# aksiksi/needle

Hardware: AMD Instinct MI355X
Metric: episode-pairs/sec (analyze+search) (higher is better)
Workload: dtype f64-certified (f32 first pass)

## Files before the change

needle_amd/csrc/common.h:

```cpp
#pragma once

#include <cstddef>
#include <cstdint>
#include <functional>
#include <string>
#include <vector>

#include "../../include/needle_hip.h"

struct ihipStream_t;

namespace needle {

struct Status {
  NeedleError code = NeedleError_Ok;
  std::string message;
  bool ok() const { return code == NeedleError_Ok; }
  static Status Ok() { return Status{}; }
  static Status Make(NeedleError c, std::string m) { return Status{c, std::move(m)}; }
};

NeedleError report(const Status &s);
void set_last_error(const std::string &m);
const char *last_error();
// ... 67 lines not shown
  uint64_t data_offset = 0;
  uint64_t frames = 0;
};
Status wav_probe(const std::string &path, WavInfo *out);
Status wav_read_frames(const std::string &path, const WavInfo &info, uint64_t first, uint64_t count, int16_t *dst);

struct StreamSpan {
  uint64_t pcm_off;
  uint64_t num_values;
  uint64_t item_off;
};

Status gpu_fingerprint_device(const int16_t *d_pcm, const std::vector<StreamSpan> &streams, int channels,
                              uint32_t step, uint32_t *d_items, bool sync, double *d_chroma_dbg = nullptr,
                              double *d_feat_dbg = nullptr, size_t descriptor_slot = 0, int pipe = -1,
                              uint32_t *zero_word = nullptr, bool *zeroed = nullptr);
Status gpu_fingerprint_streamed_device(const std::vector<const int16_t *> &pcm, const std::vector<size_t> &num_values,
                                       int channels, uint32_t step, uint32_t *d_items,
                                       const std::vector<uint64_t> &item_off);
Status gpu_fingerprint_host(const std::vector<const int16_t *> &pcm, const std::vector<size_t> &num_values,
                            int channels, uint32_t step, std::vector<std::vector<uint32_t>> *items,
                            int rate = kSampleRate);
using PcmReader = std::function<Status(size_t stream, uint64_t first_value, uint64_t num_values, int16_t *dst)>;
using StreamIssued = std::function<Status(size_t stream_index)>;
Status gpu_upload_pcm_streamed(const std::vector<size_t> &num_values, const std::vector<uint64_t> &dev_off,
                               const PcmReader &read, unsigned readers, int16_t *d_pcm, ::ihipStream_t *stream = nullptr,
                               const StreamIssued &issued = nullptr);
Status gpu_upload_pcm(const std::vector<const int16_t *> &pcm, const std::vector<size_t> &num_values,
                      const std::vector<uint64_t> &dev_off, int16_t *d_pcm, ::ihipStream_t *stream = nullptr,
                      const StreamIssued &issued = nullptr);
Status gpu_fingerprint_streamed(const std::vector<size_t> &num_values, const PcmReader &read, unsigned readers,
                                int channels, uint32_t step, std::vector<std::vector<uint32_t>> *items,
                                int rate = kSampleRate);
Status gpu_hamming_runs_device(const uint32_t *d_hashes, const NeedleHipSeq *seqs, size_t num_seqs,
                               const NeedleHipProblem *problems, size_t num_problems, uint32_t threshold,
                               NeedleHipRun *d_runs, uint32_t capacity, uint32_t *d_count, bool sync,
                               bool count_is_zero = false);
Status gpu_hamming_runs_host(const uint32_t *hashes, size_t num_hashes, const NeedleHipSeq *seqs, size_t num_seqs,
                             const NeedleHipProblem *problems, size_t num_problems, uint32_t threshold,
                             std::vector<NeedleHipRun> *runs);

uint32_t *gpu_pinned_arena_acquire(size_t words);
void gpu_pinned_arena_release(uint32_t *arena);
void gpu_prefetch_hashes(const uint32_t *hashes, size_t num_hashes);

constexpr uint64_t kDeviceEpiloguePairs = 1u << 14;
constexpr uint32_t kDeviceEpilogueRuns = 1u << 14;

Status gpu_int_valu_ceiling(double *cells_per_second);
Status gpu_scan_issued_evaluations(uint64_t *lane_evaluations, bool reset, uint64_t *head_survivors = nullptr);
void gpu_scan_last_launch(int32_t *form, uint64_t *matrix_products);
Status gpu_fingerprint_cert_stats(uint64_t out[4], bool reset);
Status gpu_fingerprint_audit_device(const int16_t *d_pcm, const std::vector<StreamSpan> &spans, int channels, uint32_t step,
                                    const uint32_t *d_items, uint64_t out[4], double *max_ratio, double *max_sigma);

struct ResampleSpan {
  uint64_t in_off;
  uint64_t n_in;
  uint64_t out_off;
};
size_t resample_out_len(size_t n_in, int rate);
Status gpu_resample_device(const int16_t *d_in, const std::vector<ResampleSpan> &spans, int channels, int rate,
                           int16_t *d_out, bool sync);
Status gpu_resample_host(const std::vector<const int16_t *> &pcm, const std::vector<size_t> &num_values, int channels,
                         int rate, std::vector<std::vector<int16_t>> *out);

struct DownmixSpan {
  const int16_t *src;
  int16_t *dst;
  uint64_t frames;
// ... 7 lines not shown
```

needle_amd/csrc/library.cpp:

```cpp
#include <hip/hip_runtime_api.h>

#include <algorithm>
#include <chrono>
#include <cstdio>
#include <cstdlib>
#include <cstring>
#include <map>
#include <new>
#include <tuple>

#include "comm.h"
#include "epilogue.h"
#include "hipctx.h"
#include "needle_core.h"

struct FrameHashes;
struct NeedleAudioComparator;

namespace needle {
const Comparator &comparator_of(const NeedleAudioComparator *c);
FrameHashes *make_frame_hashes(FrameHashesData &&d);
void fill_c_result(const VideoResult &v, NeedleHipSearchResult *r);
}

// ... 43 lines not shown
    DeviceBuffer<uint8_t> d_heads;
    uint32_t slab_runs = 0, head_runs = 0;
    int world = 0;
    void *host = nullptr;
    size_t host_bytes = 0;
    hipEvent_t searched = nullptr, done = nullptr;
    bool pending = false;
    std::vector<NeedleHipRun> merged;
    void *host_results = nullptr;
    size_t host_results_bytes = 0;
    bool device_epilogue = false, sharded = false;
    bool shape_fixed = false;
    const NeedleHipRun *last_runs = nullptr;
    size_t last_total = 0;
    DeviceBuffer<uint8_t> d_dir_send, d_dir_recv;
    DeviceBuffer<uint32_t> d_dir_counts;
    void *host_counts = nullptr;
    size_t host_counts_bytes = 0;
    std::vector<uint32_t> cap;
    bool ran_device_epilogue = false, ran_sharded = false;
    uint32_t scan_form = 0;
    bool counted = false;
    bool directed = false;
    std::vector<NeedleHipRun> fetched;
    bool fetched_valid = false;
    static size_t count_words(int world) { return ((size_t)world + 1 + 3) & ~(size_t)3; }
    uint64_t comm_bytes[4] = {0, 0, 0, 0};
    size_t slab_bytes() const { return kSlabHeader + (size_t)slab_runs * sizeof(NeedleHipRun); }
    size_t head_bytes() const { return kSlabHeader + (size_t)head_runs * sizeof(NeedleHipRun); }
  } job[2];
  static constexpr size_t kSlabHeader = 32;
  uint32_t slab_runs = 0;
  uint32_t last_max_count = 0;
  std::vector<uint32_t> dir_counts;
  int dir_world = 0;
  bool dir_unsupported = false;
  bool dir_cap_forced = false;
  size_t arena_rows = 0;
  const uint32_t *count_zeroed = nullptr;
  std::vector<uint32_t> row_len, row_ts;
  std::vector<uint64_t> row_seek, ts_tables;
  void ensure_row_tables() {
    if (row_len.size() == rows()) return;
    row_len.assign(rows(), 0);
    row_ts.assign(rows(), 0);
    row_seek.assign(rows(), 0);
    ts_tables.clear();
    std::map<uint32_t, uint32_t> offset_of;
    for (size_t row = 0; row < rows(); row++) {
      const Window &w = win[row];
      auto it = offset_of.find(w.kept);
      if (it == offset_of.end()) {
        it = offset_of.emplace(w.kept, (uint32_t)ts_tables.size()).first;
        for (const HashTs &h : timestamps(w.kept)) ts_tables.push_back(h.ts);
      }
      row_len[row] = w.kept;
      row_ts[row] = it->second;
      row_seek[row] = w.seek;
    }
  }
  ~NeedleHipLibrary() {
    for (Fetch &f : fetch) {
      if (f.host) (void)hipHostFree(f.host);
      if (f.done) (void)hipEventDestroy(f.done);
      if (f.ready) (void)hipEventDestroy(f.ready);
    }
// ... 359 lines not shown
      lib->problems_for[0] = ~(size_t)0;
    }
    std::vector<NeedleHipProblem> &problems = lib->problems;
    const bool cached = lib->problems_for[0] == first_pair && lib->problems_for[1] == num_pairs && lib->problems_for[2] == Rc;
    if (!cached) {
      lib->problems_for[0] = ~(size_t)0;
      problems.clear();
      problems.reserve(num_pairs * Rc);
      size_t i = 0, j = 0;
      if (num_pairs) pair_at(lib->n, first_pair, &i, &j);
      for (size_t p = first_pair; p < first_pair + num_pairs; p++) {
        for (size_t r = 0; r < Rc; r++) {
          if (r == 1 && (lib->win[i * R + 1].kept == 0 || lib->win[j * R + 1].kept == 0))
            return report(Status::Make(NeedleError_Unknown, "no ending hash data present"));
          const uint32_t a = lib->min_len[i * R + r], b = lib->min_len[j * R + r];
          if (a == 0 || b == 0) continue;
          problems.push_back(NeedleHipProblem{(uint32_t)(i * R + r), (uint32_t)(j * R + r), std::max(a, b),
                                              (uint32_t)(p * Rc + r)});
        }
        if (++j == lib->n) j = ++i + 1;
      }
      lib->problems_for[0] = first_pair;
      lib->problems_for[1] = num_pairs;
      lib->problems_for[2] = Rc;
    }
    for (NeedleHipLibrary::Fetch &f : lib->fetch)
      if (f.pending && (f.d_runs == d_runs || f.d_count == d_count) &&
          hipStreamWaitEvent(library_stream(), f.done, 0) != hipSuccess)
        return report(Status::Make(NeedleError_Unknown, "stream wait failed"));
    const auto t_built = std::chrono::steady_clock::now();
    const bool count_is_zero = lib->count_zeroed == d_count;
    lib->count_zeroed = nullptr;
    Status s = gpu_hamming_runs_device(lib->arena, seqs.data(), seqs.size(), problems.data(), problems.size(),
                                       cmp.hash_match_threshold(), d_runs, capacity, d_count, sync, count_is_zero);
    if (getenv("NEEDLE_HIP_TRACE"))
      std::fprintf(stderr, "[needle_hip] search enqueue: %zu problems built in %.2f ms, launched in %.2f ms\n",
                   problems.size(), std::chrono::duration<double, std::milli>(t_built - t_enter).count(),
                   std::chrono::duration<double, std::milli>(std::chrono::steady_clock::now() - t_built).count());
    return s.ok() ? NeedleError_Ok : report(s);
  });
}

enum NeedleError needle_hip_library_fetch_runs_begin(NeedleHipLibrary *lib, int slot, const NeedleHipRun *d_runs,
                                                     const uint32_t *d_count, uint32_t max_runs) {
  if (!lib || !d_runs || !d_count) return NeedleError_NullArgument;
  if (slot < 0 || slot > 1 || max_runs == 0) return NeedleError_InvalidArgument;
  return guarded([&]() -> NeedleError {
    NeedleHipLibrary::Fetch &f = lib->fetch[slot];
    if (f.pending) return report(Status::Make(NeedleError_InvalidArgument, "fetch slot still pending"));
    const size_t bytes = 16 + (size_t)max_runs * sizeof(NeedleHipRun);
    if (f.max_runs < max_runs) {
      if (f.host) (void)hipHostFree(f.host);
      f.host = nullptr;
      if (hipHostMalloc(&f.host, bytes, hipHostMallocDefault) != hipSuccess)
        return report(Status::Make(NeedleError_Unknown, "pinned allocation failed"));
      f.max_runs = max_runs;
    }
    if (!f.done && hipEventCreateWithFlags(&f.done, hipEventDisableTiming) != hipSuccess)
      return report(Status::Make(NeedleError_Unknown, "event creation failed"));
    if (!f.ready && hipEventCreateWithFlags(&f.ready, hipEventDisableTiming) != hipSuccess)
      return report(Status::Make(NeedleError_Unknown, "event creation failed"));
    hipStream_t stream = library_stream(), down = download_stream();
    if (hipEventRecord(f.ready, stream) != hipSuccess || hipStreamWaitEvent(down, f.ready, 0) != hipSuccess ||
        hipMemcpyAsync(f.host, d_count, sizeof(uint32_t), hipMemcpyDeviceToHost, down) != hipSuccess ||
        hipMemcpyAsync(static_cast<char *>(f.host) + 16, d_runs, (size_t)max_runs * sizeof(NeedleHipRun),
                       hipMemcpyDeviceToHost, down) != hipSuccess ||
        hipEventRecord(f.done, down) != hipSuccess)
// ... 152 lines not shown
}

bool device_epilogue_wanted(const NeedleHipLibrary *lib, size_t comparator_regions) {
  if (const char *e = getenv("NEEDLE_HIP_DEVICE_EPILOGUE")) return atoi(e) != 0;
  return (uint64_t)pair_count(lib->n) * comparator_regions >= kDeviceEpiloguePairs || lib->last_max_count >= kDeviceEpilogueRuns;
}

Status fetch_directed(NeedleHipLibrary::Job &j, int world, int rank) {
  if (j.fetched_valid) return Status::Ok();
  const size_t W = (size_t)world, cw = NeedleHipLibrary::Job::count_words(world);
  const uint32_t *m = static_cast<const uint32_t *>(j.host_counts);
  size_t total = 0, off = 0;
  for (size_t r = 0; r < W; r++) total += std::min(m[r * cw + 1 + (size_t)rank], j.cap[r * W + (size_t)rank]);
  j.fetched.resize(total);
  size_t at = 0;
  for (size_t r = 0; r < W; r++) {
    const uint32_t cap = j.cap[r * W + (size_t)rank], have = std::min(m[r * cw + 1 + (size_t)rank], cap);
    if (have)
      NEEDLE_HIP_TRY(hipMemcpyAsync(j.fetched.data() + at, j.d_dir_recv.ptr + off + NeedleHipLibrary::kSlabHeader,
                                    (size_t)have * sizeof(NeedleHipRun), hipMemcpyDeviceToHost, download_stream()));
    at += have;
    off += NeedleHipLibrary::kSlabHeader + (size_t)cap * sizeof(NeedleHipRun);
  }
  NEEDLE_HIP_TRY(hipStreamSynchronize(download_stream()));
  j.fetched_valid = true;
  return Status::Ok();
}

NeedleError job_search_and_gather(NeedleHipLibrary *lib, const NeedleAudioComparator *comparator, NeedleHipLibrary::Job &j) {
  const int world = comm_world(), rank = comm_rank();
  size_t pfirst = 0, pcount = 0;
  shard_range(pair_count(lib->n), world, rank, &pfirst, &pcount);
  uint8_t *mine = j.d_slabs.ptr;
  NeedleError e = needle_hip_library_search(lib, comparator, pfirst, pcount,
                                            reinterpret_cast<NeedleHipRun *>(mine + NeedleHipLibrary::kSlabHeader), j.slab_runs,
                                            reinterpret_cast<uint32_t *>(mine), false);
  if (e != NeedleError_Ok) return e;
  {
    int32_t form = 0;
    uint64_t products = 0;
    gpu_scan_last_launch(&form, &products);
    j.scan_form = (uint32_t)form;
  }
  hipStream_t stream = library_stream(), down = download_stream();
  if (hipEventRecord(j.searched, stream) != hipSuccess || hipStreamWaitEvent(down, j.searched, 0) != hipSuccess)
    return report(Status::Make(NeedleError_Unknown, "stream ordering failed"));
  const Comparator &cmp = comparator_of(comparator);
  const size_t Rc = cmp.include_endings() ? 2 : 1;
  j.device_epilogue = device_epilogue_wanted(lib, Rc) && lib->n >= 2;
  j.shape_fixed = j.device_epilogue;
  if (j.device_epilogue) {
    uint64_t shard_from = 1u << 16;
    if (const char *e = getenv("NEEDLE_HIP_SHARD_EPILOGUE_PAIRS")) shard_from = (uint64_t)std::max(1, atoi(e));
    j.sharded = world > 1 && (getenv("NEEDLE_HIP_SHARD_EPILOGUE") ? atoi(getenv("NEEDLE_HIP_SHARD_EPILOGUE")) != 0
                                                                   : (uint64_t)pair_count(lib->n) * Rc >= shard_from);
  }
  j.counted = j.directed = false;
  j.cap.clear();
  j.fetched_valid = false;
  const char *dir_env = getenv("NEEDLE_HIP_DIRECTED_RUNS");
  const bool want_directed = world > 1 && world <= 64 && j.device_epilogue && j.sharded && !lib->dir_unsupported &&
                             !(dir_env && atoi(dir_env) == 0);
  std::vector<size_t> recv_off((size_t)world, 0), recv_bytes((size_t)world, 0);
  if (want_directed) {
    const size_t W = (size_t)world;
    const bool have = lib->dir_world == world && lib->dir_counts.size() == W * W;
    std::vector<uint32_t> cap(W * W, 0u);
    if (have)
      for (size_t k = 0; k < W * W; k++) cap[k] = round_up4((uint64_t)lib->dir_counts[k] + lib->dir_counts[k] / 8 + 64);
// ... 505 lines not shown
```

needle_amd/csrc/search.hip:

```cpp
#include "epilogue.h"
#include "hipctx.h"

#include <algorithm>
#include <atomic>
#include <cstdio>
#include <cstdlib>
#include <cstring>
#include <mutex>
#include <unordered_map>

namespace needle {

namespace {

constexpr int kDiagsPerBlock = 256;
constexpr int kBandR = 7, kBandU = 3;
constexpr int kBandB = 64 * kBandR;
constexpr int kSampleW = 8;
constexpr int kSampleHead = 3;
__host__ __device__ constexpr int head_row(int k, int W, int H = kSampleHead) {
  return H == 3 ? (k == 0 ? 0 : (k == 1 ? W / 2 : W - 1)) : (k * (W - 1)) / (H - 1);
}
__host__ __device__ constexpr bool is_head_row(int s, int W, int H = kSampleHead) {
  for (int k = 0; k < H; k++)
// ... 148 lines not shown
      const uint32_t sv = src[row];
#pragma unroll
      for (int r = 0; r < R; r++) {
        const uint32_t c = (uint32_t)__popc(sv ^ W[(r + s) % R]);
        Z[r] = (c <= threshold) ? Z[r] : row;
        if (r == 0) W[s % R] = nxt[s];
      }
    }
    bool any = false;
#pragma unroll
    for (int r = 0; r < R; r++) any |= (i + K - 1 - Z[r] >= flag_len);
    if (__any(any)) checkpoint(i + K - 1);
  }
  for (; i <= i_end; i++) {
    const uint32_t sv = src[i];
#pragma unroll
    for (int r = 0; r < R; r++) {
      const uint32_t c = (uint32_t)__popc(sv ^ W[r]);
      Z[r] = (c <= threshold) ? Z[r] : i;
    }
#pragma unroll
    for (int r = 0; r + 1 < R; r++) W[r] = W[r + 1];
    W[R - 1] = lds[B + i + d_l + R];
  }
}

__device__ __forceinline__ void wave_lds_fence_search() {
  __builtin_amdgcn_fence(__ATOMIC_RELEASE, "wavefront");
  __builtin_amdgcn_wave_barrier();
  __builtin_amdgcn_fence(__ATOMIC_ACQUIRE, "wavefront");
}

template <int R, int W, bool COUNT = false, int H = kSampleHead, bool LEGACY = false>
__global__ __launch_bounds__(256) void hamming_runs_sampled_kernel(const uint32_t *__restrict__ hashes,
                                                                   const SearchProblem *__restrict__ problems,
                                                                   int num_problems, uint32_t threshold,
                                                                   NeedleHipRun *__restrict__ runs,
                                                                   uint32_t capacity, uint32_t *__restrict__ count,
                                                                   int bands_per_wave, int sparse_max,
                                                                   unsigned long long *__restrict__ eval_groups) {
  constexpr int B = 64 * R;
  unsigned long long groups = 0, survived = 0;
  extern __shared__ uint32_t lds[];
  __builtin_amdgcn_s_setprio(3);
  int lo = 0, hi = num_problems - 1;
  while (lo < hi) {
    int mid = (lo + hi + 1) >> 1;
    if (problems[mid].block_base <= blockIdx.x) lo = mid; else hi = mid - 1;
  }
  const SearchProblem pr = problems[lo];
  const int n = (int)pr.n, m = (int)pr.m;
  const uint32_t *__restrict__ src = hashes + pr.src_off;
  const uint32_t *__restrict__ dst = hashes + pr.dst_off;
  uint32_t *ldst = lds;
  for (int k = threadIdx.x; k < B; k += blockDim.x) {
    ldst[k] = 0u;
    ldst[B + m + k] = 0u;
  }
  {
    constexpr int kU = 8;
    const int nt = (int)blockDim.x;
    int k = threadIdx.x;
    for (; k + (kU - 1) * nt < m; k += kU * nt) {
      uint32_t v[kU];
#pragma unroll
      for (int u = 0; u < kU; u++) v[u] = dst[k + u * nt];
#pragma unroll
      for (int u = 0; u < kU; u++) ldst[B + k + u * nt] = v[u];
    }
    for (; k < m; k += nt) ldst[B + k] = dst[k];
  }
  const uint32_t *__restrict__ lsrc = src;
  __syncthreads();

  const int wave = __builtin_amdgcn_readfirstlane((int)(threadIdx.x >> 6));
  const int lane = (int)(threadIdx.x & 63);
  const int min_len = (int)pr.min_len;
  const int P = min_len - W + 1;
  const uint32_t bias = 31u - min(threshold, 31u);
  uint32_t held_b = 0u, held_e = 0u, held_len = 0u;
  int held = 0;
  auto flush_runs = [&]() {
    if (held == 0) return;
    uint32_t base = 0u;
    if (lane == 0) base = atomicAdd(count, (uint32_t)held);
    base = (uint32_t)__builtin_amdgcn_readfirstlane((int)base);
    if (lane < held && base + (uint32_t)lane < capacity)
      runs[base + (uint32_t)lane] = NeedleHipRun{(uint32_t)lo, held_b, held_e, held_len, 0u, 0u};
    held = 0;
  };
  auto emit_run = [&](const uint32_t b, const uint32_t e, const uint32_t len) {
    const bool mine = lane == held;
    held_b = mine ? b : held_b;
    held_e = mine ? e : held_e;
    held_len = mine ? len : held_len;
    if (++held == 64) flush_runs();
  };
  const int slots = 4 * bands_per_wave;
  const int total_bands = (n + m - 3 + B - 1) / B;
  const int nb = (total_bands + slots - 1) / slots;
  const int b_in_pair = (int)(blockIdx.x - pr.block_base);
  for (int round = 0; round < bands_per_wave; round++) {
  const int q = (round * 4 + wave + lo) % slots;
  const int band = q * nb + b_in_pair;
  const int D0 = band * B - (n - 2);
  if (band >= total_bands || D0 > m - 2) continue;
  const int i_start = max(1, 2 - D0 - B);
  const int i_end = min(n - 1, m - 1 - D0);
  const int d_l = D0 + lane * R;

  int k0 = (i_start - 1 + P - 1) / P;
  for (int w0 = 1 + k0 * P; w0 + W - 1 <= i_end; w0 += P) {
    uint32_t E[W + R - 1];
#pragma unroll
    for (int q = 0; q < W + R - 1; q++) E[q] = ldst[B + w0 + d_l + q];
    uint32_t sv[W];
#pragma unroll
    for (int s = 0; s < W; s++) sv[s] = src[w0 + s];
    bool ok[R];
    uint32_t miss[R];
#pragma unroll
    for (int r = 0; r < R; r++) miss[r] = 0u;
#pragma unroll
    for (int k = 0; k < H; k++) {
      const int s = head_row(k, W, H);
#pragma unroll
      for (int r = 0; r < R; r++) miss[r] |= (uint32_t)__popc(sv[s] ^ E[s + r]) + bias;
    }
#pragma unroll
    for (int r = 0; r < R; r++) ok[r] = miss[r] < 32u;
// ... 9 lines not shown
        const int row = e + lane;
        const bool bad = row <= fwd_limit && (uint32_t)__popc(lsrc[row] ^ ldst[B + row + d]) > threshold;
        if (COUNT) groups += 1;
        const unsigned long long mm = __ballot(bad);
        if (mm) {
          e += __ffsll((long long)mm) - 1;
          ended = true;
          break;
        }
        e += 64;
      }
      if (!ended) {
        if (fwd_limit == w0 + P + W - 1) return;
        e = ihi + 1;
      }
      const int b = e - 1;
      int a = ilo;
      int q = w0 - 1;
      while (q >= ilo) {
        const int row = q - lane;
        const bool bad = row >= ilo && (uint32_t)__popc(lsrc[row] ^ ldst[B + row + d]) > threshold;
        if (COUNT) groups += 1;
        const unsigned long long mm = __ballot(bad);
        if (mm) {
          a = q - (__ffsll((long long)mm) - 1) + 1;
          break;
        }
        q -= 64;
      }
      const int len = b - a + 1;
      if (len >= min_len) emit_run((uint32_t)b, (uint32_t)(b + d), (uint32_t)len);
    };

    unsigned long long alive[R];
    int survivors = 0;
#pragma unroll
    for (int r = 0; r < R; r++) {
      alive[r] = __ballot(ok[r]);
      survivors += __popcll(alive[r]);
    }
    if (COUNT) survived += (unsigned long long)survivors;
    if (survivors == 0) continue;
    if (!LEGACY || sparse_max < 0) {
#pragma unroll
      for (int r = 0; r < R; r++) {
        if (alive[r] == 0) continue;
        uint32_t mm = miss[r];
#pragma unroll
        for (int k = 0; k < W - H; k++) {
          const int s = tail_row(k, W, H);
          mm |= (uint32_t)__popc(sv[s] ^ E[s + r]) + bias;
        }
        if (COUNT) groups += W - H;
        unsigned long long cand = __ballot(mm < 32u);
        while (cand) {
          const int src_lane = __ffsll((long long)cand) - 1;
          cand &= cand - 1;
          resolve(D0 + src_lane * R + r);
        }
      }
      continue;
    }
    if constexpr (LEGACY) {
    if (survivors <= sparse_max) {
      constexpr int kTail = W - H;
      uint32_t sv_tail = sv[tail_row(kTail - 1, W, H)];
      int tail_off = tail_row(kTail - 1, W, H);
#pragma unroll
      for (int k = kTail - 2; k >= 0; k--) {
        sv_tail = lane == k ? sv[tail_row(k, W, H)] : sv_tail;
        tail_off = lane == k ? tail_row(k, W, H) : tail_off;
      }
#pragma unroll
      for (int r = 0; r < R; r++) {
        unsigned long long cand = alive[r];
        while (cand) {
          const int src_lane = __ffsll((long long)cand) - 1;
          cand &= cand - 1;
          const int d = D0 + src_lane * R + r;
          const int row = w0 + tail_off;
          const bool bad = (uint32_t)__popc(sv_tail ^ ldst[B + row + d]) > threshold;
          if (COUNT) groups += 1;
          if (__ballot(bad) == 0) resolve(d);
        }
      }
      continue;
    }
#pragma unroll
    for (int k = 0; k < W - H; k++) {
      const int s = tail_row(k, W, H);
// ... 104 lines not shown
    }
  }
}

struct ScanShape {
  int w = kSampleW, h = kSampleHead;
};
ScanShape scan_shape() {
  ScanShape sh;
  if (const char *e = getenv("NEEDLE_HIP_SCAN_SHAPE")) {
    int w = 0, h = 0;
    if (std::sscanf(e, "%d,%d", &w, &h) == 2 && (w == 4 || w == 8 || w == 16) && h >= 2 && h <= 4 && h < w) {
      sh.w = w;
      sh.h = h;
    }
  }
  return sh;
}
using SampledKernel = void (*)(const uint32_t *, const SearchProblem *, int, uint32_t, NeedleHipRun *, uint32_t, uint32_t *, int, int,
                               unsigned long long *);
template <bool COUNT>
SampledKernel sampled_kernel(ScanShape sh, bool legacy) {
#define NEEDLE_SHAPE(W_, H_) \
  if (sh.w == W_ && sh.h == H_) return hamming_runs_sampled_kernel<kBandR, W_, COUNT, H_, true>;
  NEEDLE_SHAPE(4, 2) NEEDLE_SHAPE(4, 3) NEEDLE_SHAPE(8, 2) NEEDLE_SHAPE(8, 4) NEEDLE_SHAPE(16, 2) NEEDLE_SHAPE(16, 3) NEEDLE_SHAPE(16, 4)
#undef NEEDLE_SHAPE
  if (legacy) return hamming_runs_sampled_kernel<kBandR, kSampleW, COUNT, kSampleHead, true>;
  return hamming_runs_sampled_kernel<kBandR, kSampleW, COUNT, kSampleHead, false>;
}

struct SearchPlan {
  std::vector<NeedleHipSeq> seqs;
  std::vector<NeedleHipProblem> problems;
  int mode[8] = {0, 0, 0, 0, 0, 0, 0, 0};
  std::vector<SearchProblem> meta;
  size_t staged = 0;
  uint64_t oversize_blocks = 0;
  uint64_t blocks = 0;
  size_t lds_bytes = 0;
  bool sampled = false, fast = false, mfma = false;
  int mfma_waves = 0, mfma_splits = 1;
  std::vector<M2ImageSeq> image_seqs;
  uint32_t image_windows = 0, image_min_len = 0;
  uint64_t mfma_products = 0;
  int bands_per_wave = 1;
  bool valid = false;
  bool matches(const NeedleHipSeq *s, size_t ns, const NeedleHipProblem *p, size_t np, const int *m) const {
    return valid && seqs.size() == ns && problems.size() == np && std::memcmp(mode, m, sizeof(mode)) == 0 &&
           std::memcmp(seqs.data(), s, ns * sizeof(NeedleHipSeq)) == 0 &&
           std::memcmp(problems.data(), p, np * sizeof(NeedleHipProblem)) == 0;
  }
};

int device_cus() {
  int cus = 256, dev = 0;
  if (hipGetDevice(&dev) == hipSuccess) (void)hipDeviceGetAttribute(&cus, hipDeviceAttributeMultiprocessorCount, dev);
  return cus > 0 ? cus : 256;
}

Status build_plan(const NeedleHipSeq *seqs, size_t num_seqs, const NeedleHipProblem *problems, size_t num_problems,
                  const int *mode, SearchPlan *plan) {
  plan->valid = false;
  std::vector<SearchProblem> &meta = plan->meta;
  meta.clear();
  meta.reserve(num_problems);
  uint64_t blocks = 0;
  for (size_t p = 0; p < num_problems; p++) {
    const NeedleHipProblem &pr = problems[p];
    if (pr.src_seq >= num_seqs || pr.dst_seq >= num_seqs)
      return Status::Make(NeedleError_InvalidArgument, "hamming_runs: problem references a missing sequence");
    if (pr.min_len == 0) return Status::Make(NeedleError_InvalidArgument, "hamming_runs: min_len must be >= 1");
    const NeedleHipSeq &a = seqs[pr.src_seq], &b = seqs[pr.dst_seq];
    if (a.len < 2 || b.len < 2) continue;
    SearchProblem m;
    m.src_off = a.offset;
    m.n = a.len;
    m.dst_off = b.offset;
    m.m = b.len;
    m.min_len = pr.min_len;
    m.tag = pr.tag;
    m.block_base = 0;
    m.pad = 0;
    meta.push_back(m);
  }
  plan->staged = 0;
  plan->oversize_blocks = 0;
  if (!meta.empty()) {
    uint32_t smallest = 0xFFFFFFFFu;
    for (const SearchProblem &m : meta) smallest = std::min(smallest, m.min_len);
    const bool generic_only = mode[0] != 0;
    const bool sampled = !generic_only && smallest >= (uint32_t)(2 * scan_shape().w - 1 + 8) && mode[1] == 0 && mode[3] == 0;
    const bool fast = !generic_only && !sampled && smallest >= (uint32_t)(kBandR * kBandU);
    const size_t lds_limit = (size_t)mode[5];
    auto windows_of = [&](const SearchProblem &m) { return (uint64_t)mfma_windows((int)m.n, (int)m.min_len, kSampleW); };
    auto same_group = [](const SearchProblem &a, const SearchProblem &b) {
      return a.dst_off == b.dst_off && a.m == b.m && a.min_len == b.min_len;
    };
    const int waves = mode[6];
    const size_t group_budget = waves == 4 ? 53760 : waves == 8 ? 81920 : 163840;
    const size_t max_members = (size_t)kM2Members;
    auto group_need = [&](const SearchProblem &a, uint64_t windows) { return m2_lds_words(a.m, windows, waves) * sizeof(uint32_t); };
    bool mfma = sampled && mode[4] == 1;
    const size_t mfma_from = 2048;
    const bool candidate = sampled && (mode[4] == 1 || (mode[4] == 2 && meta.size() >= mfma_from));
    if (candidate) {
      std::stable_sort(meta.begin(), meta.end(), [](const SearchProblem &a, const SearchProblem &b) {
        if (a.dst_off != b.dst_off) return a.dst_off < b.dst_off;
        if (a.m != b.m) return a.m < b.m;
        return a.min_len < b.min_len;
      });
      if (!mfma) {
        uint64_t windows = 0, rows = 0;
        for (size_t i = 0; i < meta.size(); i++) {
          uint64_t w = windows_of(meta[i]);
          for (size_t k = 1; k < max_members && i + 1 < meta.size() && same_group(meta[i], meta[i + 1]) &&
                             group_need(meta[i], w + windows_of(meta[i + 1])) <= group_budget; k++)
            w += windows_of(meta[++i]);
          windows += w;
          rows += (w + 31) / 32 * 32;
        }
        mfma = rows > 0 && 10 * windows >= 7 * rows;
      }
    }
    auto lds_need = [&](const SearchProblem &m) {
      if (mfma) return group_need(m, windows_of(m));
      return ((fast || sampled) ? (size_t)m.m + 2 * kBandB : (size_t)m.n + m.m) * sizeof(uint32_t);
    };
    auto mfma_packable = [&](const SearchProblem &m) { return m.m < 65536u && windows_of(m) < 8192u && m.n < (1u << 28); };
    auto stageable = [&](const SearchProblem &m) { return lds_need(m) <= lds_limit && (!mfma || mfma_packable(m)); };
    std::stable_partition(meta.begin(), meta.end(), stageable);
    size_t staged = 0;
    while (staged < meta.size() && stageable(meta[staged])) staged++;
    size_t lds_bytes = 0;
    int bands_per_wave = 1;
    size_t groups = 0;
    if (mfma) {
      const bool single = (mode[7] & 0x100) != 0;
      for (size_t i = 0; i < staged;) {
        SearchProblem &a = meta[i];
        a.pad = 0;
        uint64_t windows = windows_of(a);
        size_t k = 1;
        while (!single && k < max_members && i + k < staged && same_group(a, meta[i + k]) &&
               windows + windows_of(meta[i + k]) < 8192 &&
               group_need(a, windows + windows_of(meta[i + k])) <= group_budget) {
          windows += windows_of(meta[i + k]);
          meta[i + k].pad = 0x80000000u;
          k++;
        }
        a.pad = (uint32_t)(k - 1);
        i += k;
        groups++;
      }
    }
    if (mfma) {
      if (staged >= ((size_t)1 << 23)) return Status::Make(NeedleError_InvalidArgument, "hamming_runs: too many problems for one launch");
      size_t g = 0;
      for (size_t i = 0; i < staged; i++)
        if (!(meta[i].pad & 0x80000000u)) meta[g++].pad |= (uint32_t)i << 8;
    }
    int splits = 1;
    if (mfma && groups > 0) {
      const uint64_t slots = (uint64_t)device_cus() * (uint64_t)(waves == 4 ? 3 : waves == 8 ? 2 : 1);
      splits = (int)std::min<uint64_t>(8, std::max<uint64_t>(1, (2 * slots + groups - 1) / groups));
      if (mode[7] & 0x7F) splits = mode[7] & 0x7F;
    }
    if (fast || sampled) {
      uint64_t fb = 0, total_bands = 0;
      for (size_t i = 0; i < staged; i++) total_bands += ((uint64_t)meta[i].n + meta[i].m - 3 + kBandB - 1) / kBandB;
      if (sampled)
        while (bands_per_wave < 8 && total_bands / (4 * (uint64_t)bands_per_wave * 2) >= 16384) bands_per_wave *= 2;
      if (mode[2] > 0) bands_per_wave = mode[2];
      for (size_t i = 0; i < staged; i++) {
        SearchProblem &m = meta[i];
        m.block_base = (uint32_t)fb;
        if (mfma && (m.pad & 0x80000000u)) continue;
        const uint64_t diags = (uint64_t)m.n + m.m - 3;
        const uint64_t bands = (diags + kBandB - 1) / kBandB;
        const uint64_t per_block = 4 * (uint64_t)(sampled ? bands_per_wave : 1);
        fb += mfma ? (uint64_t)splits : (bands + per_block - 1) / per_block;
        if (mfma) {
          uint64_t windows = windows_of(m);
          for (uint32_t f = 1; f <= (m.pad & 0xFFu); f++) windows += windows_of(meta[i + f]);
          lds_bytes = std::max(lds_bytes, group_need(m, windows));
        } else {
          lds_bytes = std::max(lds_bytes, lds_need(m));
        }
      }
      blocks = fb;
    } else {
      for (size_t i = 0; i < staged; i++) {
        SearchProblem &m = meta[i];
        m.block_base = (uint32_t)blocks;
        blocks += ((uint64_t)m.n + m.m - 3 + kDiagsPerBlock - 1) / kDiagsPerBlock;
        lds_bytes = std::max(lds_bytes, lds_need(m));
      }
    }
    uint64_t ob = 0;
    for (size_t i = staged; i < meta.size(); i++) {
      meta[i].block_base = (uint32_t)ob;
      ob += ((uint64_t)meta[i].n + meta[i].m - 3 + kDiagsPerBlock - 1) / kDiagsPerBlock;
    }
    if (blocks > 0x7FFFFFFFull || ob > 0x7FFFFFFFull)
      return Status::Make(NeedleError_InvalidArgument, "hamming_runs: too many problems for one launch");
    plan->staged = staged;
    plan->oversize_blocks = ob;
    plan->sampled = sampled;
    plan->mfma = mfma;
    plan->mfma_products = 0;
    if (mfma)
      for (size_t i = 0; i < staged; i++) {
        const SearchProblem &m = meta[i];
        if (m.pad & 0x80000000u) continue;
        uint64_t w = windows_of(m);
        for (uint32_t f = 1; f <= (m.pad & 0xFFu); f++) w += windows_of(meta[i + f]);
        if (w > 0 && m.m >= (uint32_t)kSampleW + 1) {
          uint64_t col_blocks = ((uint64_t)m.m - kSampleW) / 32 + 1;
          col_blocks = (col_blocks + kM2ColBlocks - 1) / kM2ColBlocks * kM2ColBlocks;
          plan->mfma_products += (w + 31) / 32 * col_blocks * (kM2Heads / 2);
        }
      }
    plan->image_seqs.clear();
    plan->image_windows = plan->image_min_len = 0;
    if (mfma && staged > 0 && !(mode[7] & 0x200)) {
      bool one = true;
      for (size_t i = 1; i < staged && one; i++) one = meta[i].min_len == meta[0].min_len;
      if (one) {
        std::unordered_map<uint64_t, uint32_t> first_of;
        uint64_t total = 0;
        for (size_t i = 0; i < staged; i++) {
          const uint64_t key = ((uint64_t)meta[i].src_off << 32) | meta[i].n;
          auto it = first_of.find(key);
          if (it == first_of.end()) {
            const uint32_t w = (uint32_t)windows_of(meta[i]);
            it = first_of.emplace(key, (uint32_t)total).first;
            plan->image_seqs.push_back(M2ImageSeq{meta[i].src_off, meta[i].n, (uint32_t)total, w});
            total += w;
          }
          meta[i].block_base = it->second;
        }
        if (total == 0 || total * kM2ImageWords * sizeof(uint32_t) > ((uint64_t)1 << 31)) {
// ... 9 lines not shown
    plan->mfma_splits = splits;
    plan->bands_per_wave = bands_per_wave;
    plan->lds_bytes = lds_bytes;
  }
  plan->blocks = blocks;
  plan->seqs.assign(seqs, seqs + num_seqs);
  plan->problems.assign(problems, problems + num_problems);
  std::memcpy(plan->mode, mode, sizeof(plan->mode));
  plan->valid = true;
  return Status::Ok();
}

int mfma_request(uint32_t threshold) {
  if (threshold > 15u || scan_shape().w != kSampleW || getenv("NEEDLE_HIP_SCAN_SHAPE") || getenv("NEEDLE_HIP_SCAN_COUNT")) return 0;
  const char *e = getenv("NEEDLE_HIP_SCAN_MFMA");
  if (!e) return 2;
  return atoi(e) != 0 ? 1 : 0;
}

int mfma_waves() {
  int waves = 8;
  if (const char *e = getenv("NEEDLE_HIP_MFMA_WAVES")) {
    const int w = atoi(e);
    if (w == 4 || w == 8 || w == 12 || w == 16) waves = w;
  }
  return waves;
}
using Mfma2Kernel = void (*)(const uint32_t *, const SearchProblem *, int, uint32_t, NeedleHipRun *, uint32_t, uint32_t *, int, const uint32_t *);
Mfma2Kernel mfma2_kernel(int waves) {
  return waves == 4 ? hamming_runs_mfma2_kernel<kSampleW, 4, 3> : waves == 16 ? hamming_runs_mfma2_kernel<kSampleW, 16, 4>
       : waves == 12 ? hamming_runs_mfma2_kernel<kSampleW, 12, 3> : hamming_runs_mfma2_kernel<kSampleW, 8, 4>;
}

std::atomic<int32_t> g_last_form{0};
std::atomic<uint64_t> g_last_products{0};

struct SearchWorkspace {
  DeviceBuffer<SearchProblem> problems;
  PinnedStage stage;
  DescriptorUpload<SearchProblem> upload;
  SearchPlan plan;
  DeviceBuffer<M2ImageSeq> image_seqs;
  PinnedStage image_stage;
  DescriptorUpload<M2ImageSeq> image_upload;
  DeviceBuffer<uint32_t> images;
  bool lds_attr_set = false;
  unsigned long long *eval_groups = nullptr;
};
std::mutex g_ws_mu;
std::map<int, SearchWorkspace *> g_ws;

SearchWorkspace *workspace() {
  int dev = 0;
  (void)hipGetDevice(&dev);
  std::lock_guard<std::mutex> lock(g_ws_mu);
  auto it = g_ws.find(dev);
  if (it != g_ws.end()) return it->second;
  SearchWorkspace *w = new SearchWorkspace();
  g_ws[dev] = w;
  return w;
}


}

void gpu_scan_last_launch(int32_t *form, uint64_t *matrix_products) {
  *form = g_last_form.load();
  *matrix_products = g_last_products.load();
}

Status gpu_hamming_runs_device(const uint32_t *d_hashes, const NeedleHipSeq *seqs, size_t num_seqs,
                               const NeedleHipProblem *problems, size_t num_problems, uint32_t threshold,
                               NeedleHipRun *d_runs, uint32_t capacity, uint32_t *d_count, bool sync, bool count_is_zero) {
  std::lock_guard<std::recursive_mutex> gpu_lock(gpu_mutex());
  Status s = ensure_device();
  if (!s.ok()) return s;
  hipStream_t stream = library_stream();
  if (!count_is_zero) NEEDLE_HIP_TRY(hipMemsetAsync(d_count, 0, sizeof(uint32_t), stream));
  const int mode[8] = {getenv("NEEDLE_HIP_GENERIC_SEARCH") != nullptr, getenv("NEEDLE_HIP_BAND_SEARCH") != nullptr,
                       getenv("NEEDLE_HIP_BANDS_PER_WAVE") ? std::max(1, atoi(getenv("NEEDLE_HIP_BANDS_PER_WAVE"))) : 0,
                       threshold > 31u,
                       mfma_request(threshold),
                       getenv("NEEDLE_HIP_SEARCH_LDS_LIMIT") ? std::max(1, atoi(getenv("NEEDLE_HIP_SEARCH_LDS_LIMIT"))) : 160 * 1024,
                       mfma_waves(),
                       (getenv("NEEDLE_HIP_MFMA_SPLITS") ? std::max(1, std::min(64, atoi(getenv("NEEDLE_HIP_MFMA_SPLITS")))) : 0) |
                           (getenv("NEEDLE_HIP_MFMA_SINGLE") ? 0x100 : 0) | (getenv("NEEDLE_HIP_MFMA_NO_IMAGES") ? 0x200 : 0)};
  SearchWorkspace *ws = workspace();
  SearchPlan &plan = ws->plan;
  const bool reuse = plan.matches(seqs, num_seqs, problems, num_problems, mode);
  if (!reuse && !(s = build_plan(seqs, num_seqs, problems, num_problems, mode, &plan)).ok()) return s;
  const std::vector<SearchProblem> &meta = plan.meta;
  const uint64_t blocks = plan.blocks;
  const size_t lds_bytes = plan.lds_bytes;
  const bool sampled = plan.sampled, fast = plan.fast;
  const int bands_per_wave = plan.bands_per_wave;
  if (!meta.empty()) {
    if (!(reuse && ws->upload.resident_at == ws->problems.ptr && ws->problems.ptr) &&
        !(s = ws->upload.put(&ws->problems, &ws->stage, meta, stream)).ok())
      return s;
    if (lds_bytes > 64 * 1024 && !ws->lds_attr_set) {
      NEEDLE_HIP_TRY(hipFuncSetAttribute(reinterpret_cast<const void *>(hamming_runs_kernel<true>),
                                         hipFuncAttributeMaxDynamicSharedMemorySize, 160 * 1024));
      NEEDLE_HIP_TRY(hipFuncSetAttribute(reinterpret_cast<const void *>(hamming_runs_band_kernel<kBandR, kBandU>),
                                         hipFuncAttributeMaxDynamicSharedMemorySize, 160 * 1024));
      for (int w : {4, 8, 12, 16})
        NEEDLE_HIP_TRY(hipFuncSetAttribute(reinterpret_cast<const void *>(mfma2_kernel(w)),
                                           hipFuncAttributeMaxDynamicSharedMemorySize, 160 * 1024));
      for (int w : {4, 8, 16})
        for (int h : {2, 3, 4}) {
          if (h >= w) continue;
          for (bool legacy : {false, true}) {
            NEEDLE_HIP_TRY(hipFuncSetAttribute(reinterpret_cast<const void *>(sampled_kernel<false>(ScanShape{w, h}, legacy)),
                                               hipFuncAttributeMaxDynamicSharedMemorySize, 160 * 1024));
            NEEDLE_HIP_TRY(hipFuncSetAttribute(reinterpret_cast<const void *>(sampled_kernel<true>(ScanShape{w, h}, legacy)),
                                               hipFuncAttributeMaxDynamicSharedMemorySize, 160 * 1024));
          }
        }
      ws->lds_attr_set = true;
    }
    const int staged = (int)plan.staged, oversize = (int)(meta.size() - plan.staged);
    g_last_form.store(staged > 0 ? (sampled ? (plan.mfma ? 4 : 3) : fast ? 2 : 1) : 1);
    g_last_products.store(staged > 0 && plan.mfma ? plan.mfma_products : 0);
    if (staged > 0) {
      KernelTimer timer("hamming_runs");
      if (sampled) {
        int sparse_max = -1;
        if (const char *e = getenv("NEEDLE_HIP_SPARSE_MAX")) sparse_max = std::max(0, atoi(e));
        if (getenv("NEEDLE_HIP_SCAN_COUNT")) {
          if (!ws->eval_groups) {
            NEEDLE_HIP_TRY(hipMalloc((void **)&ws->eval_groups, 2 * sizeof(unsigned long long)));
            NEEDLE_HIP_TRY(hipMemsetAsync(ws->eval_groups, 0, 2 * sizeof(unsigned long long), stream));
          }
          hipLaunchKernelGGL(sampled_kernel<true>(scan_shape(), sparse_max >= 0), dim3((uint32_t)blocks), dim3(256), lds_bytes, stream, d_hashes,
                             ws->problems.ptr, staged, threshold, d_runs, capacity, d_count, bands_per_wave, sparse_max,
                             ws->eval_groups);
        } else if (plan.mfma) {
          const uint32_t *images = nullptr;
          if (!plan.image_seqs.empty()) {
            if (!(s = ws->image_upload.put(&ws->image_seqs, &ws->image_stage, plan.image_seqs, stream)).ok() ||
                !(s = ws->images.reserve((size_t)plan.image_windows * kM2ImageWords)).ok())
              return s;
            const uint32_t grid = (uint32_t)std::min<uint64_t>(8192, ((uint64_t)plan.image_windows * kM2Rows + 255) / 256);
            hipLaunchKernelGGL(m2_window_images_kernel<kSampleW>, dim3(grid), dim3(256), 0, stream, d_hashes, ws->image_seqs.ptr,
                               (int)plan.image_seqs.size(), plan.image_windows, plan.image_min_len, ws->images.ptr);
            images = ws->images.ptr;
          }
          hipLaunchKernelGGL(mfma2_kernel(plan.mfma_waves), dim3((uint32_t)blocks), dim3(64 * plan.mfma_waves),
                             lds_bytes, stream, d_hashes, ws->problems.ptr, staged, threshold, d_runs, capacity, d_count,
                             plan.mfma_splits, images);
#if NEEDLE_M2_LAB & 8
          {
            unsigned long long c[8], z[8] = {};
            (void)hipStreamSynchronize(stream);
            (void)hipMemcpyFromSymbol(c, HIP_SYMBOL(m2_dbg), sizeof c);
            (void)hipMemcpyToSymbol(HIP_SYMBOL(m2_dbg), z, sizeof z);
            fprintf(stderr, "m2 counts: resolve calls %llu, trips %llu, mismatches handled %llu, walks continued %llu, extra forward trips %llu, "
                            "windows past the tail rows %llu, items %llu, windows past the head rows %llu\n", c[0], c[1], c[2], c[3], c[4], c[5], c[6], c[7]);
          }
#endif
        } else {
          hipLaunchKernelGGL(sampled_kernel<false>(scan_shape(), sparse_max >= 0), dim3((uint32_t)blocks), dim3(256), lds_bytes, stream, d_hashes,
                             ws->problems.ptr, staged, threshold, d_runs, capacity, d_count, bands_per_wave, sparse_max,
                             (unsigned long long *)nullptr);
        }
      }
      else if (fast)
        hipLaunchKernelGGL((hamming_runs_band_kernel<kBandR, kBandU>), dim3((uint32_t)blocks), dim3(256), lds_bytes,
                           stream, d_hashes, ws->problems.ptr, staged, threshold, d_runs, capacity, d_count);
      else
        hipLaunchKernelGGL(hamming_runs_kernel<true>, dim3((uint32_t)blocks), dim3(256), lds_bytes, stream, d_hashes,
                           ws->problems.ptr, staged, 0u, threshold, d_runs, capacity, d_count);
    }
    if (oversize > 0) {
      KernelTimer timer("hamming_runs_unstaged");
      hipLaunchKernelGGL(hamming_runs_kernel<false>, dim3((uint32_t)plan.oversize_blocks), dim3(256), 0, stream, d_hashes,
                         ws->problems.ptr + staged, oversize, (uint32_t)staged, threshold, d_runs, capacity, d_count);
    }
    {
      KernelTimer timer("simhash_runs");
      hipLaunchKernelGGL(simhash_runs_kernel, dim3(2048), dim3(256), 0, stream, d_hashes, ws->problems.ptr, d_runs,
                         capacity, d_count);
    }
    NEEDLE_HIP_TRY(hipGetLastError());
  }
  if (sync) NEEDLE_HIP_TRY(hipStreamSynchronize(stream));
  return Status::Ok();
}

Status gpu_scan_issued_evaluations(uint64_t *lane_evaluations, bool reset, uint64_t *head_survivors) {
  std::lock_guard<std::recursive_mutex> gpu_lock(gpu_mutex());
  Status s = ensure_device();
  if (!s.ok()) return s;
  SearchWorkspace *ws = workspace();
  unsigned long long groups[2] = {0, 0};
  hipStream_t stream = library_stream();
  if (ws->eval_groups) {
    NEEDLE_HIP_TRY(hipMemcpyAsync(groups, ws->eval_groups, sizeof(groups), hipMemcpyDeviceToHost, stream));
    if (reset) NEEDLE_HIP_TRY(hipMemsetAsync(ws->eval_groups, 0, sizeof(groups), stream));
    NEEDLE_HIP_TRY(hipStreamSynchronize(stream));
  }
  *lane_evaluations = (uint64_t)groups[0] * 64u;
  if (head_survivors) *head_survivors = (uint64_t)groups[1];
  return Status::Ok();
}

namespace {
struct HostCallBuffers {
  DeviceBuffer<uint32_t> d_hashes, d_count;
  DeviceBuffer<NeedleHipRun> d_runs;
  void *pinned = nullptr;
  size_t pinned_bytes = 0;
  uint32_t *arena = nullptr;
  size_t arena_words = 0;
// ... 260 lines not shown
```

Baseline: 711,400.

## Add opt-in pipelined MFMA scan plan and size simhash grid from last run count

Adds a ScanHints struct that passes whether the STFT stream is active and the previous run count into the search launch. A new env-gated pipelined mode forces the MFMA scan with 4 waves, a smaller LDS group budget and fewer splits so the scan can share the device with concurrent fingerprinting. Separately, the simhash_runs grid is shrunk from a fixed 2048 blocks to a size derived from the previous run count, which cuts idle block launch overhead. The grid heuristic relies on the previous count and on the kernel's grid-stride loop to stay correct if runs grow.

```diff
diff --git a/needle_amd/csrc/common.h b/needle_amd/csrc/common.h
--- a/needle_amd/csrc/common.h
+++ b/needle_amd/csrc/common.h
@@ -123,10 +123,14 @@
 Status gpu_fingerprint_streamed(const std::vector<size_t> &num_values, const PcmReader &read, unsigned readers,
                                 int channels, uint32_t step, std::vector<std::vector<uint32_t>> *items,
                                 int rate = kSampleRate);
+struct ScanHints {
+  bool pipelined = false;
+  uint32_t last_runs = 0;
+};
 Status gpu_hamming_runs_device(const uint32_t *d_hashes, const NeedleHipSeq *seqs, size_t num_seqs,
                                const NeedleHipProblem *problems, size_t num_problems, uint32_t threshold,
                                NeedleHipRun *d_runs, uint32_t capacity, uint32_t *d_count, bool sync,
-                               bool count_is_zero = false);
+                               bool count_is_zero = false, const ScanHints &hints = ScanHints());
 Status gpu_hamming_runs_host(const uint32_t *hashes, size_t num_hashes, const NeedleHipSeq *seqs, size_t num_seqs,
                              const NeedleHipProblem *problems, size_t num_problems, uint32_t threshold,
                              std::vector<NeedleHipRun> *runs);
diff --git a/needle_amd/csrc/library.cpp b/needle_amd/csrc/library.cpp
--- a/needle_amd/csrc/library.cpp
+++ b/needle_amd/csrc/library.cpp
@@ -99,6 +99,7 @@
   static constexpr size_t kSlabHeader = 32;
   uint32_t slab_runs = 0;
   uint32_t last_max_count = 0;
+  ScanHints scan_hints;
   std::vector<uint32_t> dir_counts;
   int dir_world = 0;
   bool dir_unsupported = false;
@@ -524,7 +525,7 @@
     const bool count_is_zero = lib->count_zeroed == d_count;
     lib->count_zeroed = nullptr;
     Status s = gpu_hamming_runs_device(lib->arena, seqs.data(), seqs.size(), problems.data(), problems.size(),
-                                       cmp.hash_match_threshold(), d_runs, capacity, d_count, sync, count_is_zero);
+                                       cmp.hash_match_threshold(), d_runs, capacity, d_count, sync, count_is_zero, lib->scan_hints);
     if (getenv("NEEDLE_HIP_TRACE"))
       std::fprintf(stderr, "[needle_hip] search enqueue: %zu problems built in %.2f ms, launched in %.2f ms\n",
                    problems.size(), std::chrono::duration<double, std::milli>(t_built - t_enter).count(),
@@ -743,9 +744,12 @@
   size_t pfirst = 0, pcount = 0;
   shard_range(pair_count(lib->n), world, rank, &pfirst, &pcount);
   uint8_t *mine = j.d_slabs.ptr;
+  lib->scan_hints.pipelined = stft_stream() != nullptr;
+  lib->scan_hints.last_runs = lib->last_max_count;
   NeedleError e = needle_hip_library_search(lib, comparator, pfirst, pcount,
                                             reinterpret_cast<NeedleHipRun *>(mine + NeedleHipLibrary::kSlabHeader), j.slab_runs,
                                             reinterpret_cast<uint32_t *>(mine), false);
+  lib->scan_hints = ScanHints();
   if (e != NeedleError_Ok) return e;
   {
     int32_t form = 0;
diff --git a/needle_amd/csrc/search.hip b/needle_amd/csrc/search.hip
--- a/needle_amd/csrc/search.hip
+++ b/needle_amd/csrc/search.hip
@@ -537,13 +537,13 @@
 struct SearchPlan {
   std::vector<NeedleHipSeq> seqs;
   std::vector<NeedleHipProblem> problems;
-  int mode[8] = {0, 0, 0, 0, 0, 0, 0, 0};
+  int mode[10] = {};
   std::vector<SearchProblem> meta;
   size_t staged = 0;
   uint64_t oversize_blocks = 0;
   uint64_t blocks = 0;
   size_t lds_bytes = 0;
-  bool sampled = false, fast = false, mfma = false;
+  bool sampled = false, fast = false, mfma = false, pipelined = false;
   int mfma_waves = 0, mfma_splits = 1;
   std::vector<M2ImageSeq> image_seqs;
   uint32_t image_windows = 0, image_min_len = 0;
@@ -601,20 +601,22 @@
     auto same_group = [](const SearchProblem &a, const SearchProblem &b) {
       return a.dst_off == b.dst_off && a.m == b.m && a.min_len == b.min_len;
     };
-    const int waves = mode[6];
-    const size_t group_budget = waves == 4 ? 53760 : waves == 8 ? 81920 : 163840;
+    int waves = mode[6];
+    size_t group_budget = waves == 4 ? 53760 : waves == 8 ? 81920 : 163840;
     const size_t max_members = (size_t)kM2Members;
     auto group_need = [&](const SearchProblem &a, uint64_t windows) { return m2_lds_words(a.m, windows, waves) * sizeof(uint32_t); };
     bool mfma = sampled && mode[4] == 1;
     const size_t mfma_from = 2048;
-    const bool candidate = sampled && (mode[4] == 1 || (mode[4] == 2 && meta.size() >= mfma_from));
+    const bool pipe_request = sampled && mode[8] > 0 && mode[4] == 2;
+    bool pipe = false;
+    const bool candidate = sampled && (mode[4] == 1 || pipe_request || (mode[4] == 2 && meta.size() >= mfma_from));
     if (candidate) {
       std::stable_sort(meta.begin(), meta.end(), [](const SearchProblem &a, const SearchProblem &b) {
         if (a.dst_off != b.dst_off) return a.dst_off < b.dst_off;
         if (a.m != b.m) return a.m < b.m;
         return a.min_len < b.min_len;
       });
-      if (!mfma) {
+      if (!mfma && meta.size() >= mfma_from) {
         uint64_t windows = 0, rows = 0;
         for (size_t i = 0; i < meta.size(); i++) {
           uint64_t w = windows_of(meta[i]);
@@ -625,6 +627,11 @@
           rows += (w + 31) / 32 * 32;
         }
         mfma = rows > 0 && 10 * windows >= 7 * rows;
+      }
+      if (!mfma && pipe_request) {
+        mfma = pipe = true;
+        waves = 4;
+        group_budget = (size_t)mode[8];
       }
     }
     auto lds_need = [&](const SearchProblem &m) {
@@ -668,7 +675,10 @@
     if (mfma && groups > 0) {
       const uint64_t slots = (uint64_t)device_cus() * (uint64_t)(waves == 4 ? 3 : waves == 8 ? 2 : 1);
       splits = (int)std::min<uint64_t>(8, std::max<uint64_t>(1, (2 * slots + groups - 1) / groups));
+      if (pipe)
+        splits = (int)std::min<uint64_t>(8, std::max<uint64_t>(1, (uint64_t)device_cus() / groups));
       if (mode[7] & 0x7F) splits = mode[7] & 0x7F;
+      if (pipe && mode[9] > 0) splits = mode[9];
     }
     if (fast || sampled) {
       uint64_t fb = 0, total_bands = 0;
@@ -712,6 +722,7 @@
     plan->oversize_blocks = ob;
     plan->sampled = sampled;
     plan->mfma = mfma;
+    plan->pipelined = mfma && pipe;
     plan->mfma_products = 0;
     if (mfma)
       for (size_t i = 0; i < staged; i++) {
@@ -787,6 +798,9 @@
        : waves == 12 ? hamming_runs_mfma2_kernel<kSampleW, 12, 3> : hamming_runs_mfma2_kernel<kSampleW, 8, 4>;
 }
 
+constexpr int kPipeGroupLds = 81920;
+constexpr uint32_t kSimhashMinGrid = 64;
+
 std::atomic<int32_t> g_last_form{0};
 std::atomic<uint64_t> g_last_products{0};
 
@@ -826,20 +840,24 @@
 
 Status gpu_hamming_runs_device(const uint32_t *d_hashes, const NeedleHipSeq *seqs, size_t num_seqs,
                                const NeedleHipProblem *problems, size_t num_problems, uint32_t threshold,
-                               NeedleHipRun *d_runs, uint32_t capacity, uint32_t *d_count, bool sync, bool count_is_zero) {
+                               NeedleHipRun *d_runs, uint32_t capacity, uint32_t *d_count, bool sync, bool count_is_zero,
+                               const ScanHints &hints) {
   std::lock_guard<std::recursive_mutex> gpu_lock(gpu_mutex());
   Status s = ensure_device();
   if (!s.ok()) return s;
   hipStream_t stream = library_stream();
   if (!count_is_zero) NEEDLE_HIP_TRY(hipMemsetAsync(d_count, 0, sizeof(uint32_t), stream));
-  const int mode[8] = {getenv("NEEDLE_HIP_GENERIC_SEARCH") != nullptr, getenv("NEEDLE_HIP_BAND_SEARCH") != nullptr,
+  const bool pipe = hints.pipelined && getenv("NEEDLE_HIP_SCAN_PIPELINED") && atoi(getenv("NEEDLE_HIP_SCAN_PIPELINED")) != 0;
+  const int mode[10] = {getenv("NEEDLE_HIP_GENERIC_SEARCH") != nullptr, getenv("NEEDLE_HIP_BAND_SEARCH") != nullptr,
                        getenv("NEEDLE_HIP_BANDS_PER_WAVE") ? std::max(1, atoi(getenv("NEEDLE_HIP_BANDS_PER_WAVE"))) : 0,
                        threshold > 31u,
                        mfma_request(threshold),
                        getenv("NEEDLE_HIP_SEARCH_LDS_LIMIT") ? std::max(1, atoi(getenv("NEEDLE_HIP_SEARCH_LDS_LIMIT"))) : 160 * 1024,
                        mfma_waves(),
                        (getenv("NEEDLE_HIP_MFMA_SPLITS") ? std::max(1, std::min(64, atoi(getenv("NEEDLE_HIP_MFMA_SPLITS")))) : 0) |
-                           (getenv("NEEDLE_HIP_MFMA_SINGLE") ? 0x100 : 0) | (getenv("NEEDLE_HIP_MFMA_NO_IMAGES") ? 0x200 : 0)};
+                           (getenv("NEEDLE_HIP_MFMA_SINGLE") ? 0x100 : 0) | (getenv("NEEDLE_HIP_MFMA_NO_IMAGES") ? 0x200 : 0),
+                       !pipe ? 0 : getenv("NEEDLE_HIP_PIPE_LDS") ? std::max(16384, std::min(160 * 1024, atoi(getenv("NEEDLE_HIP_PIPE_LDS")))) : kPipeGroupLds,
+                       pipe && getenv("NEEDLE_HIP_PIPE_SPLITS") ? std::max(1, std::min(64, atoi(getenv("NEEDLE_HIP_PIPE_SPLITS")))) : 0};
   SearchWorkspace *ws = workspace();
   SearchPlan &plan = ws->plan;
   const bool reuse = plan.matches(seqs, num_seqs, problems, num_problems, mode);
@@ -874,7 +892,7 @@
       ws->lds_attr_set = true;
     }
     const int staged = (int)plan.staged, oversize = (int)(meta.size() - plan.staged);
-    g_last_form.store(staged > 0 ? (sampled ? (plan.mfma ? 4 : 3) : fast ? 2 : 1) : 1);
+    g_last_form.store(staged > 0 ? (sampled ? (plan.pipelined ? 5 : plan.mfma ? 4 : 3) : fast ? 2 : 1) : 1);
     g_last_products.store(staged > 0 && plan.mfma ? plan.mfma_products : 0);
     if (staged > 0) {
       KernelTimer timer("hamming_runs");
@@ -932,8 +950,12 @@
                          ws->problems.ptr + staged, oversize, (uint32_t)staged, threshold, d_runs, capacity, d_count);
     }
     {
+      uint32_t grid = 2048;
+      if (hints.last_runs)
+        grid = (uint32_t)std::min<uint64_t>(2048, std::max<uint64_t>(kSimhashMinGrid, ((uint64_t)hints.last_runs + hints.last_runs / 4 + 64 + 3) / 4));
+      if (const char *e = getenv("NEEDLE_HIP_SIMHASH_GRID")) grid = (uint32_t)std::max(1, std::min(2048, atoi(e)));
       KernelTimer timer("simhash_runs");
-      hipLaunchKernelGGL(simhash_runs_kernel, dim3(2048), dim3(256), 0, stream, d_hashes, ws->problems.ptr, d_runs,
+      hipLaunchKernelGGL(simhash_runs_kernel, dim3(grid), dim3(256), 0, stream, d_hashes, ws->problems.ptr, d_runs,
                          capacity, d_count);
     }
     NEEDLE_HIP_TRY(hipGetLastError());
```

Result: no change. 701,200, median of 4 (-1.4%).

## Resolve runs in constant-hash regions with block-level extent walks

Applied to the files above, without the earlier changes.

When all sampled source hashes in a window are identical, candidate diagonals are resolved together. The code walks the constant-hash extents in source and destination once, then derives each run's endpoints from those extents. Diagonals it cannot settle fall back to the per-diagonal resolve path, and the candidate loop now iterates per lane over a pending bitmask. This targets repeated per-diagonal walks in long runs of identical hashes such as silence, at the cost of heavier control flow and an added waves_per_eu occupancy hint that may force register spills.

```diff
diff --git a/needle_amd/csrc/search.hip b/needle_amd/csrc/search.hip
--- a/needle_amd/csrc/search.hip
+++ b/needle_amd/csrc/search.hip
@@ -204,7 +204,7 @@
 }
 
 template <int R, int W, bool COUNT = false, int H = kSampleHead, bool LEGACY = false>
-__global__ __launch_bounds__(256) void hamming_runs_sampled_kernel(const uint32_t *__restrict__ hashes,
+__global__ __launch_bounds__(256) __attribute__((amdgpu_waves_per_eu(8))) void hamming_runs_sampled_kernel(const uint32_t *__restrict__ hashes,
                                                                    const SearchProblem *__restrict__ problems,
                                                                    int num_problems, uint32_t threshold,
                                                                    NeedleHipRun *__restrict__ runs,
@@ -268,6 +268,18 @@
     held_len = mine ? len : held_len;
     if (++held == 64) flush_runs();
   };
+  auto walk = [&](const uint32_t *p, const int start, const int step, const int limit, const uint32_t key, const uint32_t tol) {
+    for (int k = 0; k < limit; k += 64) {
+      const int idx = k + lane;
+      const bool stop = idx < limit && (uint32_t)__popc(p[start + step * idx] ^ key) > tol;
+      if (COUNT) groups += 1;
+      const unsigned long long mm = __ballot(stop);
+      if (mm) return k + __ffsll((long long)mm) - 1;
+    }
+    return limit;
+  };
+  uint32_t st_h = 0u;
+  int st_a = 1, st_e = 0;
   const int slots = 4 * bands_per_wave;
   const int total_bands = (n + m - 3 + B - 1) / B;
   const int nb = (total_bands + slots - 1) / slots;
@@ -343,6 +355,102 @@
       if (len >= min_len) emit_run((uint32_t)b, (uint32_t)(b + d), (uint32_t)len);
     };
 
+    auto block_pass = [&](uint32_t &pend, const uint32_t h) {
+      if (!(h == st_h && w0 >= st_a && w0 + W <= st_e)) {
+        st_h = h;
+        st_a = w0 - walk(lsrc, w0 - 1, -1, w0, h, 0u);
+        st_e = w0 + W + walk(lsrc, w0 + W, 1, n - w0 - W, h, 0u);
+      }
+      const int cap = w0 + P + W - 1;
+      const uint32_t *dstp = ldst + B;
+      uint32_t todo = 0u;
+#pragma unroll 1
+      for (int r = 0; r < R; r++) {
+        const int d = d_l + r;
+        const bool in = w0 >= (d < 0 ? 1 - d : 1) && w0 + W - 1 <= min(n - 1, m - 1 - d);
+        todo |= ((pend >> r) & 1u) && in ? 1u << r : 0u;
+      }
+      pend &= todo;
+      unsigned long long lanes;
+      while ((lanes = __ballot(todo != 0u)) != 0ull) {
+        const int ll = __ffsll((long long)lanes) - 1;
+        const int rl = __ffs(__builtin_amdgcn_readlane((int)todo, ll)) - 1;
+        const int cl = w0 + D0 + ll * R + rl;
+        const uint32_t h2 = (uint32_t)__builtin_amdgcn_readfirstlane((int)dstp[cl]);
+        const int b0 = cl - walk(dstp, cl - 1, -1, cl, h2, 0u);
+        const int b1 = cl + 1 + walk(dstp, cl + 1, 1, m - cl - 1, h2, 0u);
+        uint32_t grp = 0u;
+        bool nfs = false, nfd = false, nbs = false, nbd = false;
+#pragma unroll 1
+        for (int r = 0; r < R; r++) {
+          const int d = d_l + r;
+          if (!((todo >> r) & 1u) || w0 + d < b0 || w0 + d + W > b1) continue;
+          grp |= 1u << r;
+          const int ilo = d < 0 ? 1 - d : 1, lim = min(min(n - 1, m - 1 - d), cap) + 1;
+          const int rd = b1 - d, yd = b0 - d;
+          if (min(st_e, rd) >= lim && lim == cap + 1) continue;
+          nfs |= st_e < rd && st_e < lim;
+          nfd |= rd < st_e && rd < lim;
+          nbs |= st_a > yd && st_a > ilo;
+          nbd |= yd > st_a && yd > ilo;
+        }
+        todo &= ~grp;
+        if (ll == (int)lane) todo &= ~(1u << rl);
+        pend &= ~grp;
+        const int fs = __ballot(nfs) ? walk(lsrc, st_e, 1, min(n, cap + 1) - st_e, h2, threshold) : 0;
+        const int fd = __ballot(nfd) ? walk(dstp, b1, 1, min(m - b1, P), h, threshold) : 0;
+        const int bs = __ballot(nbs) ? walk(lsrc, st_a - 1, -1, st_a - 1, h2, threshold) : 0;
+        const int bd = __ballot(nbd) ? walk(dstp, b0 - 1, -1, b0 - 1, h, threshold) : 0;
+#pragma unroll 1
+        for (int r = 0; r < R; r++) {
+          const int d = d_l + r;
+          bool emit = false, corner = false;
+          int e = 0, a = 0;
+          if ((grp >> r) & 1u) {
+            const int ilo = d < 0 ? 1 - d : 1, ihi = min(n - 1, m - 1 - d), lim = min(ihi, cap) + 1;
+            const int rd = b1 - d, yd = b0 - d;
+            if (min(st_e, rd) >= lim) {
+              e = lim;
+            } else if (st_e < rd) {
+              const int t = st_e + fs;
+              e = t < rd ? min(t, lim) : lim;
+              corner = t >= rd && rd < lim;
+            } else if (rd < st_e) {
+              const int t = rd + fd;
+              e = t < st_e ? min(t, lim) : lim;
+              corner = t >= st_e && st_e < lim;
+            } else {
+              corner = true;
+            }
+            const bool next = e == cap + 1 && cap <= ihi;
+            if (corner || next) {
+            } else if (max(st_a, yd) <= ilo) {
+              a = ilo;
+            } else if (st_a > yd) {
+              const int t = st_a - bs;
+              a = max(t, ilo);
+              corner |= t <= yd && yd > ilo;
+            } else if (yd > st_a) {
+              const int t = yd - bd;
+              a = max(t, ilo);
+              corner |= t <= st_a && st_a > ilo;
+            } else {
+              corner = true;
+            }
+            emit = !corner && !next && e - a >= min_len;
+          }
+          pend |= corner ? 1u << r : 0u;
+          unsigned long long em = __ballot(emit);
+          while (em) {
+            const int l = __ffsll((long long)em) - 1;
+            em &= em - 1;
+            const int bl = __builtin_amdgcn_readlane(e - 1, l), dl = __builtin_amdgcn_readlane(d, l);
+            emit_run((uint32_t)bl, (uint32_t)(bl + dl), (uint32_t)__builtin_amdgcn_readlane(e - a, l));
+          }
+        }
+      }
+    };
+
     unsigned long long alive[R];
     int survivors = 0;
 #pragma unroll
@@ -353,6 +461,7 @@
     if (COUNT) survived += (unsigned long long)survivors;
     if (survivors == 0) continue;
     if (!LEGACY || sparse_max < 0) {
+      uint32_t pend = 0u;
 #pragma unroll
       for (int r = 0; r < R; r++) {
         if (alive[r] == 0) continue;
@@ -363,10 +472,20 @@
           mm |= (uint32_t)__popc(sv[s] ^ E[s + r]) + bias;
         }
         if (COUNT) groups += W - H;
-        unsigned long long cand = __ballot(mm < 32u);
-        while (cand) {
-          const int src_lane = __ffsll((long long)cand) - 1;
-          cand &= cand - 1;
+        pend |= mm < 32u ? 1u << r : 0u;
+      }
+      bool flat = true;
+#pragma unroll
+      for (int s = 1; s < W; s++) flat = flat && sv[s] == sv[0];
+      if (flat && __ballot(pend != 0u)) block_pass(pend, sv[0]);
+      unsigned long long lanes = __ballot(pend != 0u);
+      while (lanes) {
+        const int src_lane = __ffsll((long long)lanes) - 1;
+        lanes &= lanes - 1;
+        uint32_t bits = (uint32_t)__builtin_amdgcn_readlane((int)pend, src_lane);
+        while (bits) {
+          const int r = __ffs(bits) - 1;
+          bits &= bits - 1;
           resolve(D0 + src_lane * R + r);
         }
       }
```

Measured after the change: 714,000 before, 702,900 after (median of 2 runs). About the same (-1.6%).
